# DataZooDE/anofox-forecast

Hardware: AMD Instinct MI355X
Metric: series/sec fit+forecast, AutoETS h=28 on M5-shape batches (higher is better)
Workload: dtype f64

## Files before the change

### anofox-forecast_amd/csrc/ets_group_kernel.hpp

```cpp
#pragma once
#include "fit_units.hpp"

namespace anofox {

template <int ID, int MSG> constexpr int group_member_ms()
{
    if constexpr (SpecOf<ID>::s == 0) return 0;
    else if constexpr (MSG == 12 && !SpecOf<ID>::Cfg::ADDITIVE) return -1;
    else return MSG;
}
template <int ID, int MSG> constexpr bool group_member_k4() { return SpecOf<ID>::Cfg::ADDITIVE && (group_member_ms<ID, MSG>() == 0 || group_member_ms<ID, MSG>() == 7); }

template <class YT, int... IDS> struct GroupTraits {
    static constexpr bool OK = ((RoundTraits<typename SpecOf<IDS>::Cfg, YT>::WAVES == RoundTraits<typename SpecOf<0>::Cfg, YT>::WAVES &&
                                 RoundTraits<typename SpecOf<IDS>::Cfg>::WPB == 1 && !RoundTraits<typename SpecOf<IDS>::Cfg>::PARK) && ...);
};

template <class YT> constexpr int group_waves = RoundTraits<typename SpecOf<0>::Cfg, YT>::WAVES;

template <int ID, int MSG, class YT>
__device__ __forceinline__ void ets_group_slot(const FitArgs &a, const int k4, const int vblock, const int vgrid, double *const lds)
{
    using Cfg = typename SpecOf<ID>::Cfg;
    constexpr int MS = group_member_ms<ID, MSG>();
    if constexpr (SpecOf<ID>::s != 0 && MSG == 0) return;
    else {
        if constexpr (group_member_k4<ID, MSG>())
            if (k4) { ets_round_body<Cfg, MS, 3, true, YT>(a, vblock, vgrid, 0, lds); return; }
        ets_round_body<Cfg, MS, 3, false, YT>(a, vblock, vgrid, 0, lds);
    }
}

template <int MSG, class YT, int... IDS>
__global__ __launch_bounds__(NM_BLOCK, group_waves<YT>) void ets_group_round_kernel(const FitArgs *__restrict__ tab, const GroupRoundArgs g)
{
    extern __shared__ double lds_all[];
    const int b = (int)blockIdx.x;
    int k = 0;
    while (k + 1 < g.n_slots && b >= g.start[k + 1]) k++;
    const FitArgs &a = *(const FitArgs *)((const __attribute__((address_space(4))) FitArgs *)tab + k);
    const int vblock = b - g.start[k], vgrid = g.start[k + 1] - g.start[k], id = g.spec[k], k4 = g.k4[k];
    (void)((id == IDS && (ets_group_slot<IDS, MSG, YT>(a, k4, vblock, vgrid, lds_all), true)) || ...);
}

template <int MSG, class YT, int... IDS>
void ets_group_round_launch(const FitArgs *tab, const GroupRoundArgs &g, int m, hipStream_t stream)
{
    const int blocks = g.start[g.n_slots];
    if (blocks <= 0) return;
    size_t lds_doubles = 0;
    ((lds_doubles = std::max(lds_doubles, (size_t)nm_lds_doubles<SpecOf<IDS>::Cfg::DIM>() +
                                              (group_member_ms<IDS, MSG>() == -1 ? (size_t)m * NM_BLOCK : 0))), ...);
    const size_t lds_bytes = sizeof(double) * lds_doubles;
    if (lds_bytes > 48 * 1024)
        anofox_check_attr(hipFuncSetAttribute((const void *)ets_group_round_kernel<MSG, YT, IDS...>, hipFuncAttributeMaxDynamicSharedMemorySize, (int)lds_bytes));
    hipLaunchKernelGGL((ets_group_round_kernel<MSG, YT, IDS...>), dim3(blocks), dim3(NM_BLOCK), lds_bytes, stream, tab, g);
}

template <int MSG, int... IDS> GroupLaunchFn group_launcher_of_yt(int yt)
{
    if constexpr (!GroupTraits<double, IDS...>::OK || !GroupTraits<float, IDS...>::OK) return nullptr;
    else {
        if (yt == YT_U16) {
            if constexpr (ets_u16_variant(MSG) && GroupTraits<unsigned short, IDS...>::OK) return &ets_group_round_launch<MSG, unsigned short, IDS...>;
            else return nullptr;
        }
        if (yt == YT_F32) return &ets_group_round_launch<MSG, float, IDS...>;
        return &ets_group_round_launch<MSG, double, IDS...>;
    }
}
template <int... IDS> GroupLaunchFn group_launcher_of(int m, int yt)
{
    if (m <= 1) return group_launcher_of_yt<0, IDS...>(yt);
    if (m == 7) return group_launcher_of_yt<7, IDS...>(yt);
    constexpr bool ring12 = ((SpecOf<IDS>::s != 0 && SpecOf<IDS>::Cfg::ADDITIVE) || ...);
    if (m == 12 && ring12) return group_launcher_of_yt<12, IDS...>(yt);
    if (m > ETS_LDS_PERIOD) return group_launcher_of_yt<-2, IDS...>(yt);
    return group_launcher_of_yt<-1, IDS...>(yt);
}

}
```

### anofox-forecast_amd/csrc/fit_group_additive.hip

```cpp
#include "ets_group_kernel.hpp"
namespace anofox {
GroupLaunchFn fit_group_additive(int m, int yt) { return group_launcher_of<0, 1, 3, 4, 6, 7>(m, yt); }
}
```

### anofox-forecast_amd/csrc/fit_group_damped_mul.hip

```cpp
#include "ets_group_kernel.hpp"
namespace anofox {
GroupLaunchFn fit_group_damped_mul(int m, int yt) { return group_launcher_of<12, 13, 14, 27, 29>(m, yt); }
}
```

### anofox-forecast_amd/csrc/fit_group_general.hip

```cpp
#include "ets_group_kernel.hpp"
namespace anofox {
GroupLaunchFn fit_group_general(int m, int yt) { return group_launcher_of<2, 5, 8, 9, 10, 11, 15, 17, 18, 20, 21, 23, 24, 26>(m, yt); }
}
```

### anofox-forecast_amd/csrc/host_api.hip

```cpp
#include <hip/hip_runtime.h>

#include <algorithm>
#include <cctype>
#include <atomic>
#include <memory>
#include <unordered_map>
#include <chrono>
#include <cmath>
#include <condition_variable>
#include <mutex>
#include <cstdio>
#include <cstdlib>
#include <cstring>
#include <limits>
#include <map>
#include <stdexcept>
#include <string>
#include <system_error>
#include <thread>
#include <vector>

#include "classic_device.hpp"
#include "host_semantics.hpp"
#include "kernels.hpp"
// ... 765 lines not shown
        }
        b->yc_cells = cells;
    }
    if (!b->d_misfit) b->d_misfit = dalloc<unsigned int>(2);
    HIPCHECK(hipMemsetAsync(b->d_misfit, 0, 2 * sizeof(unsigned int), st));
    launch_compact_block(b->d_y, b->ld, d_len, (int)b->n, (int)std::max<size_t>(b->t_max, 1), b->d_yc32, b->d_yc16, b->d_misfit, st);
    b->h_misfit[0] = b->h_misfit[1] = 1u;
    HIPCHECK(hipMemcpyAsync(b->h_misfit, b->d_misfit, sizeof b->h_misfit, hipMemcpyDeviceToHost, st));
    return true;
}
void compact_storage_decide(AnofoxHipBatch *b, bool pending, hipStream_t st, int m)
{
    b->y_type = YT_F64;
    if (!pending) return;
    HIPCHECK(hipStreamSynchronize(st));
    const bool u16_kernels = b->d_m_col == nullptr && (m <= 1 || m == 7);
    if (b->h_misfit[1] == 0u && b->tun.compact != 1 && u16_kernels) b->y_type = YT_U16;
    else if (b->h_misfit[0] == 0u) b->y_type = YT_F32;
}

static_assert(N_GROUP_CLASSES == FIT_GROUP_CLASSES && GROUP_DAMPED_MUL == 0 && GROUP_GENERAL == 1 && GROUP_ADDITIVE == 2, "host_fit_schedule.hpp names the group classes by number");
void launch_fit_slots(AnofoxHipBatch *b, const std::vector<int> &specs, const int32_t *d_len, int m, bool skip_constant,
                      hipStream_t st)
{
    const size_t n = b->n, ld = b->ld, n_spec = specs.size();
    HIPCHECK(hipEventRecord(b->ev_fit0, st));
    const bool merged = b->d_m_col != nullptr;
    const int yt = b->y_type;
    const void *ybase = yt == YT_F32 ? (const void *)b->d_yc32 : (yt == YT_U16 ? (const void *)b->d_yc16 : (const void *)b->d_y);
    const int ybytes = yt == YT_F32 ? 4 : (yt == YT_U16 ? 2 : 8);
    const int lds_limit = merged ? ETS_MERGED_LDS_PERIOD : ETS_LDS_PERIOD;
    std::vector<FitLaunchers> fns_of(n_spec);
    GroupLaunchFn group_fn[N_GROUP_CLASSES];
    FitScheduleInput in;
    in.n = n; in.ld = ld; in.t_max = b->t_max; in.m = m;
    for (size_t k = 0; k < n_spec; k++) {
        const int id = specs[k], ms = spec_season(id) != 0 ? m : 1;
        fns_of[k] = ets_fit_launcher(id, (merged && ms != 1) ? (ms > lds_limit ? ETS_PERLANE_HBM : ETS_PERLANE_LDS) : ms, yt);
        if (!fns_of[k].round_seq || !fns_of[k].round_spec || !fns_of[k].round_auto || !fns_of[k].final) throw HipFail{"no kernel for ETS spec id " + std::to_string(id)};
        in.specs.push_back(FitSpec{id, spec_has_mult(id), spec_trend_idx(id) == 4, spec_season(id) != 0, fns_of[k].round_k4 && fns_of[k].round_auto_k4,
                                   fns_of[k].nm_scratch_per_wg, ets_group_class(id)});
    }
    for (int c = 0; c < N_GROUP_CLASSES; c++) { group_fn[c] = ets_group_launcher(c, m, yt); in.group_launcher[c] = group_fn[c] != nullptr; }
    in.live_pos = b->live_pos; in.live_all = b->live_all; in.use_pos = b->use_pos; in.none_pos = b->none_pos;
    in.fixed_params = b->fixed_params; in.merged = merged; in.fp64 = yt == YT_F64; in.use_gather = b->use_gather; in.gather_budget = b->gather_budget;
    in.seq_rounds = b->seq_rounds; in.seq_rounds_env = b->seq_rounds_env;
    in.spec_below = b->spec_below; in.spec_below_md = b->spec_below_md; in.spec2_below = b->spec2_below; in.spec2_below_md = b->spec2_below_md;
    in.n_lanes = std::min<int>(N_AUX_STREAMS, b->n_slots_cap);
    {
        const Tunables &t = b->tun;
        in.budgets = t.budgets; in.k4 = t.k4; in.k4_top = t.k4_top; in.k4_top_below = t.k4_top_below;
        in.fill_policy = t.fill_policy; in.fill_target = t.fill_target; in.fill_late_div = t.fill_late_div; in.fill_s2_div = t.fill_s2_div;
        in.top_boost_n = t.top_boost_n; in.top_boost_pct = t.top_boost_pct; in.prio_top = t.prio_top;
        in.group_launch = t.group_launch; in.group_split = t.group_split; in.dm_head_rounds = t.dm_head_rounds; in.gather_cols = t.gather_cols;
    }
    in.lim = FitLimits{NM_BLOCK, NM_K, GROUP_MAX_SLOTS, N_AUX_STREAMS, TINY_BATCH_PROBLEMS, lds_limit, 2 * 1024 * 64};
    const FitSchedule plan = plan_fit_schedule(in);
    if (!plan.error.empty()) throw HipFail{plan.error};
    auto spec_stream = [&](size_t oi) -> hipStream_t { return plan.inline_stream ? st : b->aux[plan.stream_of[oi]]; };
    std::vector<FitArgs> args(n_spec);
    std::vector<FitLaunchers> fns(n_spec);
    for (size_t oi = 0; oi < n_spec; oi++) {
        const size_t k = plan.order[oi];
        const int id = specs[k];
        auto &lane = b->lanes[plan.lane_of[oi]];
        const int se = spec_season(id), ti = spec_trend_idx(id);
        const int tt = ti == 0 ? 0 : (ti <= 2 ? 1 : 2);
        FitArgs &a = args[oi];
        a = FitArgs{};
        a.y = (const double *)ybase; a.ld = ld; a.len = d_len; a.n_series = (int)n; a.t_rows = (int)std::max<size_t>(b->t_max, 1);
        a.m = se != 0 ? m : 1; a.h = b->h;
        a.l0 = b->d_l0 + (size_t)(se * 3 + tt) * ld;
        a.b0 = b->d_b0 + (size_t)(se * 3 + tt) * ld;
        a.fig = se == 1 ? b->d_fig_add : (se == 2 ? b->d_fig_mul : nullptr);
        a.fig_ld = ld;
        a.flags = b->d_flags;
        a.need_positive = spec_has_mult(id) ? 1 : 0;
        a.skip_constant = skip_constant ? 1 : 0;
        a.n_param = spec_n_param(id, a.m);
        a.aicc = b->d_aicc + k * ld;
        a.yhat = b->d_yhat_slots + k * n * (size_t)b->h;
        a.status = b->d_status_slots + k * ld;
        a.evals = b->d_evals_slots + k * ld;
        a.iters = b->d_iters_slots + k * ld;
        a.passes = b->d_passes_slots + k * ld;
        a.st = lane.st;
        a.ring_scratch = nullptr;
// ... 137 lines not shown
        hipStream_t sg = b->aux[plan.groups[g].stream];
        if (r == 0) {
            int32_t *zero[GROUP_MAX_SLOTS] = {};
            for (size_t k = 0; k < slots.size(); k++) zero[k] = b->lanes[plan.lane_of[slots[k]]].cnt;
            launch_group_zero3((int)slots.size(), zero, sg);
        }
        GroupCompactArgs gc{}; gc.n_series = (int)n;
        GroupGatherArgs gg{}; gg.t_max = (int)b->t_max; gg.elem_bytes = ybytes; gg.y = ybase; gg.ld = ld;
        int gg_cols = 0;
        GroupRoundArgs ga{};
        ga.n_slots = (int)slots.size();
        for (int k = 0; k < ga.n_slots; k++) {
            const size_t oi = slots[(size_t)k];
            const RoundStep &s = plan.steps[oi][(size_t)r];
            auto &lane = b->lanes[plan.lane_of[oi]];
            if (s.source == SRC_POSITIVE) retire_nonpositive(oi, sg);
            else if (s.source == SRC_COMPACTED) {
                const int c = gc.n_slots++;
                gc.prev[c] = (r == 1) ? nullptr : lane.map[(r - 1) & 1]; gc.n_prev[c] = (r == 1) ? nullptr : lane.cnt + ((r - 1) % 3); gc.done[c] = lane.st.done;
                gc.next[c] = lane.map[r & 1]; gc.n_next[c] = lane.cnt + (r % 3); gc.n_clear[c] = lane.cnt + ((r + 1) % 3);
                if (b->use_gather && lane.ybuf) {
                    const int j = gg.n_slots++;
                    gg.series_of[j] = lane.map[r & 1]; gg.n_active[j] = lane.cnt + (r % 3);
                    gg.out[j] = lane.ybuf; gg.ld_out[j] = lane.ybuf_cols; gg.cap[j] = (int)lane.ybuf_cols;
                    gg_cols = std::max(gg_cols, (int)std::min<size_t>(n, lane.ybuf_cols));
                }
            }
            ga.spec[k] = specs[plan.order[oi]];
            ga.k4[k] = s.k4 ? 1 : 0;
            ga.start[k + 1] = ga.start[k] + s.workgroups;
        }
        if (gc.n_slots > 0) launch_group_compact(gc, sg);
        if (gg.n_slots > 0) launch_group_gather(gg, gg_cols, sg);
        group_fn[plan.groups[g].cls](b->d_group_tab + (size_t)r * plan.n_slots + plan.slot_of[slots[0]], ga, m, sg);
        b->fit_launches++;
    };
    if (plan.head_rounds > 0) {
        for (int r = 0; r < plan.head_rounds; r++) {
            if (plan.grouped) enqueue_group_round(r, 0);
            else for (size_t oi = 0; oi < n_spec; oi++) if (plan.head[oi]) enqueue_round(r, oi);
        }
        LAUNCHCHECK("ETS fit head rounds");
        if (plan.grouped) {
            HIPCHECK(hipEventRecord(b->ev_join[0], b->aux[0]));
            for (size_t g = 1; g < plan.groups.size(); g++) HIPCHECK(hipStreamWaitEvent(b->aux[plan.groups[g].stream], b->ev_join[0], 0));
        } else {
            for (size_t od = 0; od < n_spec; od++) if (plan.head[od]) HIPCHECK(hipEventRecord(b->ev_join[plan.stream_of[od]], spec_stream(od)));
            for (size_t oi = 0; oi < n_spec; oi++) {
                if (plan.dead[oi] || plan.head[oi]) continue;
                for (size_t od = 0; od < n_spec; od++) if (plan.head[od]) HIPCHECK(hipStreamWaitEvent(spec_stream(oi), b->ev_join[plan.stream_of[od]], 0));
            }
        }
    }
    for (int r = 0; r < plan.total_rounds; r++) {
        const bool ahead = r < plan.head_rounds;
        if (plan.grouped) {
            for (size_t g = 0; g < plan.groups.size(); g++) if (!(ahead && plan.head[plan.groups[g].slots[0]])) enqueue_group_round(r, g);
        } else
            for (size_t oi = 0; oi < n_spec; oi++) if (!(ahead && plan.head[oi])) enqueue_round(r, oi);
        LAUNCHCHECK("ETS fit round");
    }
    if (b->fixed_params && n_spec == 1) HIPCHECK(hipEventRecord(b->ev_fit0, spec_stream(0)));
    for (size_t oi = 0; oi < n_spec; oi++) if (!plan.dead[oi]) fns[oi].final(args[oi], spec_stream(oi));
    if (b->fixed_params && n_spec == 1) HIPCHECK(hipEventRecord(b->ev_fit1, spec_stream(0)));
    LAUNCHCHECK("ETS final pass");
    for (int q : plan.fork_streams) {
        HIPCHECK(hipEventRecord(b->ev_join[q], b->aux[q]));
// ... 6979 lines not shown
```

### anofox-forecast_amd/csrc/host_fit_schedule.hpp

```cpp
#pragma once

enum RoundKind { RK_SEQ, RK_SPEC, RK_SPEC2, RK_AUTO, RK_K4, RK_AUTO_K4 };
enum SeriesSource { SRC_ALL, SRC_POSITIVE, SRC_COMPACTED };
constexpr int FIT_GROUP_CLASSES = 3;

struct FitLimits {
    int nm_block, nm_k;
    int group_max_slots;
    int n_aux_streams;
    int tiny_batch_problems;
    int lds_period;
    int64_t resident_lanes;
};

struct FitSpec {
    int id;
    bool has_mult, damped_mul, seasonal;
    bool has_k4;
    size_t nm_scratch_per_wg;
    int group_class;
};

struct FitScheduleInput {
    size_t n = 0, ld = 0, t_max = 0;
    int m = 1;
    std::vector<FitSpec> specs;
    int32_t live_pos = -1, live_all = -1;
    bool use_pos = false, none_pos = false, fixed_params = false, merged = false, fp64 = true, use_gather = false;
    double gather_budget = 0.0;
    int seq_rounds = 3, seq_rounds_env = -1;
    int spec_below = 8192, spec_below_md = 8192, spec2_below = 1024, spec2_below_md = 2048;
    int n_lanes = 1;
    std::vector<int> budgets;
    int k4 = -1, k4_top = 1, k4_top_below = 20480;
    int fill_policy = 1, fill_target = 150, fill_late_div = 2, fill_s2_div = 16;
    int top_boost_n = 0, top_boost_pct = 200, prio_top = 0;
    int group_launch = 1, group_split = 1, dm_head_rounds = 0, gather_cols = 0;
    bool group_launcher[FIT_GROUP_CLASSES] = {false, false, false};
    FitLimits lim{};
};

struct RoundStep {
    int kind;
    int budget, budget_seq;
    int spec_below, spec2_below;
    int wave_prio;
    int source;
    int workgroups;
    bool k4;
};

struct FitGroup { std::vector<size_t> slots; int stream; int cls; };

struct FitSchedule {
    std::string error;
    std::vector<size_t> order;
    std::vector<int> stream_of, lane_of;
    bool inline_stream = false;
    std::vector<int> fork_streams;
    std::vector<char> dead, k4, fill_spec4, head;
    bool fill_mode = false, tiny = false, grouped = false;
    int total_rounds = 0, head_rounds = 0;
    std::vector<FitGroup> groups;
    std::vector<size_t> slot_of;
    size_t n_slots = 0;
    size_t scratch_workgroups = 0;
    std::vector<size_t> gather_cols;
    std::vector<std::vector<RoundStep>> steps;
};

inline int fit_cost(int id)
{
    static const int measured[30] = { 3, 8, 14,  7, 13, 27,  17, 29, 41,  14, 26, 22,  63, 92, 84,
                                      7, 0, 15,  18, 0, 29,  33, 0, 48,  16, 0, 28,  65, 0, 95};
    return (id >= 0 && id < 30 && measured[id] > 0) ? measured[id] : 1;
}
inline double work(const FitScheduleInput &in, const FitSpec &s)
{
    const double live = (in.live_all >= 0 && s.has_mult) ? (double)in.live_pos : (in.live_all >= 0 ? (double)in.live_all : 1.0);
    return (double)fit_cost(s.id) * (live + 1.0);
}
inline int64_t live_problems(const FitScheduleInput &in, const FitSpec &s)
{
    return (s.has_mult && in.live_pos >= 0) ? (int64_t)in.live_pos : (in.live_all >= 0 ? (int64_t)in.live_all : (int64_t)in.n);
}
inline bool tiny_batch(const FitScheduleInput &in) { return (uint64_t)in.n * in.specs.size() <= (uint64_t)in.lim.tiny_batch_problems; }
inline size_t widest_launch_workgroups(const FitScheduleInput &in)
{
    const size_t n = in.n;
    return std::max<size_t>((n + 15) / 16, std::min<size_t>(n, tiny_batch(in) ? n : (size_t)std::max(in.spec2_below, in.spec2_below_md)));
}
inline int step_workgroups(const FitScheduleInput &in, const RoundStep &s)
{
    const int64_t n = (int64_t)in.n, per_spec = in.lim.nm_block / in.lim.nm_k;
    const int64_t g_seq = (n + in.lim.nm_block - 1) / in.lim.nm_block;
    if (s.kind == RK_SEQ || s.kind == RK_K4) return (int)g_seq;
// ... 82 lines not shown
            if (c < 0 || c >= FIT_GROUP_CLASSES || !in.group_launcher[c] || spec(oi).nm_scratch_per_wg != 0) p.grouped = false;
            else of_class[c].push_back(oi);
        }
        auto add = [&](const std::vector<size_t> &sl, int c) {
            if (sl.empty()) return;
            if (sl.size() > (size_t)in.lim.group_max_slots) p.error = "launch_fit_slots: more specs in one group than GROUP_MAX_SLOTS";
            p.groups.push_back(FitGroup{sl, 0, c});
        };
        auto add_class = [&](int c, bool split) {
            if (!split) { add(of_class[c], c); return; }
            std::vector<size_t> half[2];
            double w[2] = {0.0, 0.0};
            for (size_t oi : of_class[c]) {
                const int j = w[1] < w[0] ? 1 : 0;
                half[j].push_back(oi); w[j] += work(in, spec(oi));
            }
            add(half[0], c); add(half[1], c);
        };
        if (p.grouped) {
            add_class(0, in.group_split == 1);
            add_class(1, in.group_split == 2);
            add_class(2, false);
            if (!p.error.empty()) return p;
            p.grouped = !p.groups.empty();
        }
        for (size_t g = 0; g < p.groups.size(); g++) {
            const bool dm = spec(p.groups[g].slots[0]).damped_mul;
            p.groups[g].stream = dm ? (int)g : in.lim.n_aux_streams - 1 - (int)g;
            for (size_t oi : p.groups[g].slots) { p.stream_of[oi] = p.groups[g].stream; p.slot_of[oi] = p.n_slots++; }
        }
        if (p.grouped) for (size_t oi = 0; oi < n_spec; oi++) if (p.dead[oi]) p.stream_of[oi] = p.groups[0].stream;
    }
    if (p.grouped) for (const FitGroup &g : p.groups) p.fork_streams.push_back(g.stream);
    else if (!p.inline_stream) for (int i = 0; i < in.n_lanes; i++) p.fork_streams.push_back(i);
    p.head.assign(n_spec, 0);
    if (in.dm_head_rounds > 0 && p.total_rounds > 0 && !p.tiny && !p.inline_stream) {
        size_t n_dm = 0, n_rest = 0;
        if (p.grouped) {
            if (p.groups.size() > 1 && p.groups[0].stream == 0 && spec(p.groups[0].slots[0]).damped_mul) {
                for (size_t oi : p.groups[0].slots) p.head[oi] = 1;
                n_dm = n_rest = 1;
            }
        } else
            for (size_t oi = 0; oi < n_spec; oi++) {
                if (p.dead[oi]) continue;
                if (spec(oi).damped_mul) { p.head[oi] = 1; n_dm++; } else n_rest++;
            }
        if (n_dm && n_rest) p.head_rounds = std::min(in.dm_head_rounds, p.total_rounds);
        else p.head.assign(n_spec, 0);
    }
    p.steps.resize(n_spec);
    for (size_t oi = 0; oi < n_spec; oi++) {
        if (p.dead[oi]) continue;
        const FitSpec &sp = spec(oi);
        const int64_t live = live_problems(in, sp);
        const int s2 = sp.damped_mul ? in.spec2_below_md : in.spec2_below;
        for (int r = 0; r < p.total_rounds; r++) {
            RoundStep s{};
            s.wave_prio = (int)oi < in.prio_top ? std::max(1, 3 - (int)oi) : 0;
            s.spec_below = -1; s.spec2_below = -1;
            s.source = (p.tiny || (r == 0 && !(in.use_pos && sp.has_mult))) ? SRC_ALL : (r == 0 ? SRC_POSITIVE : SRC_COMPACTED);
            if (p.tiny) {
                s.kind = RK_SPEC2; s.budget = 1 << 30;
            } else if (p.fill_mode && !p.k4[oi]) {
                s.budget = BUDGET[r];
                if (r == 0) {
                    s.kind = p.fill_spec4[oi] ? RK_SPEC : RK_SEQ;
                    if (!p.fill_spec4[oi]) s.budget = (BUDGET[r] * 7) / 4;
                } else {
                    s.kind = RK_AUTO; s.budget_seq = (BUDGET[r] * 7) / 4;
                    s.spec_below = p.fill_spec4[oi] ? unconditional : (int)std::max<int64_t>(64, live / std::max(1, in.fill_late_div));
                    s.spec2_below = (int)std::max<int64_t>(32, std::min<int64_t>(s2 > 0 ? s2 : 32, live / std::max(1, in.fill_s2_div)));
                }
            } else if (p.k4[oi]) {
                const int sb = ((int)oi < in.k4_top && in.k4_top_below > 0) ? in.k4_top_below : in.spec_below;
                s.budget = BUDGET[r];
                if (r == 0) s.kind = live > sb ? RK_K4 : RK_SPEC;
                else { s.kind = RK_AUTO_K4; s.budget_seq = BUDGET[r]; s.spec_below = sb; s.spec2_below = s2 > 0 ? s2 : -1; }
            } else if (r == 0 || in.seq_rounds_env >= 0 || in.seq_rounds == 0) {
                const bool spec_mode = r >= in.seq_rounds;
                s.budget = spec_mode ? BUDGET[r] : (BUDGET[r] * 7) / 4;
                if (spec_mode && r > 0 && s2 > 0) { s.kind = RK_AUTO; s.budget_seq = s.budget; s.spec_below = unconditional; s.spec2_below = s2; }
                else s.kind = spec_mode ? RK_SPEC : RK_SEQ;
            } else {
                s.kind = RK_AUTO; s.budget = BUDGET[r]; s.budget_seq = (BUDGET[r] * 7) / 4;
                s.spec_below = sp.damped_mul ? in.spec_below_md : in.spec_below;
                s.spec2_below = s2 > 0 ? s2 : -1;
                if ((int)oi < in.top_boost_n) {
                    s.spec_below = (int)std::min<int64_t>(unconditional, (int64_t)s.spec_below * in.top_boost_pct / 100);
                    if (s.spec2_below > 0) s.spec2_below = (int)std::min<int64_t>(unconditional, (int64_t)s.spec2_below * in.top_boost_pct / 100);
                }
            }
            if (s.kind != RK_AUTO && s.kind != RK_AUTO_K4) s.budget_seq = s.budget;
            s.k4 = s.kind == RK_K4 || s.kind == RK_AUTO_K4;
            if (p.grouped) {
                if (s.kind == RK_SPEC) s.spec_below = unconditional;
                else if (s.kind == RK_SPEC2) { p.error = "launch_fit_slots: the one-wave-per-problem round of a tiny batch has no group form"; return p; }
            }
            s.workgroups = step_workgroups(in, s);
            if (p.grouped && sp.seasonal && in.m > in.lim.lds_period && (size_t)s.workgroups > p.scratch_workgroups) {
                p.error = "launch_fit_slots: the seasonal-ring scratch does not cover a group slot"; return p;
            }
            p.steps[oi].push_back(s);
        }
    }
    return p;
}
```

### anofox-forecast_amd/csrc/host_resources.hpp

```cpp
#pragma once

constexpr int N_AUX_STREAMS = 32;

struct HipFail { std::string msg; bool oom = false; };
void report_hip_failure(AnofoxError *out_error, const HipFail &f)
{
    if (f.oom) anofox::set_error(out_error, ALLOCATION_ERROR, "Allocation error: " + f.msg);
    else anofox::set_error(out_error, INTERNAL_ERROR, "Internal error: " + f.msg);
}
#define HIPCHECK(expr)                                                                             \
    do {                                                                                           \
        hipError_t _e = (expr);                                                                    \
        if (_e != hipSuccess) throw HipFail{std::string(#expr) + ": " + hipGetErrorString(_e), _e == hipErrorOutOfMemory};    \
    } while (0)

#define LAUNCHCHECK(what)                                                                          \
    do {                                                                                           \
        hipError_t _e = hipGetLastError();                                                         \
        if (_e != hipSuccess) throw HipFail{std::string("kernel launch failed (") + (what) + "): " + hipGetErrorString(_e), false};    \
    } while (0)

constexpr int32_t STATUS_NOT_COMPUTED = -1;

struct Tunables {
    std::vector<int> budgets{24, 24, 24, 24, 24, 24, 48, 48, 96, 96, 192, 1024};
    int seq_rounds = -1;
    int gather_cols = 0;
    int gather = -1;
    int spec_below = 8192;
    int spec_below_md = 8192;
    int spec2_below = 1024;
    int spec2_below_md = 2048;
    int k4 = -1;
    int k4_top = 1, k4_top_below = 20480;
    std::string wave_trace;
    int compact = -1;
    int fill_policy = 1;
    int fill_target = 150;
    int fill_late_div = 2;
    int fill_s2_div = 16;
    int top_boost_n = 0, top_boost_pct = 200;
    int prio_top = 0;
    int group_launch = 1;
    int group_split = 1;
    int dm_head_rounds = 0;
    bool merge_periods = true;
    int part_threads = 16;
    int pack_threads = 0;
    bool timing = false;
    int arima_trace = 0;
    double arima_lookahead = 6.0;
    int arima_lookahead_depth = 2;
    double arima_spec_factor = 4.0;
    double arima_shared_chunk_rounds = 1.0;
    int arima_prep_lanes = 64;
    int arima_queue_sort = 1;
    int arima_refit_budget = 100;
    static std::map<std::string, std::string> tune_map()
    {
        std::map<std::string, std::string> kv;
        const char *e = std::getenv("ANOFOX_HIP_TUNE");
        if (!e) return kv;
        std::string all(e);
        for (size_t pos = 0; pos < all.size();) {
            size_t end = all.find(';', pos);
            if (end == std::string::npos) end = all.size();
            const std::string item = all.substr(pos, end - pos);
            const size_t eq = item.find('=');
            if (eq != std::string::npos) {
                std::string k = item.substr(0, eq), v = item.substr(eq + 1);
                while (!k.empty() && k.front() == ' ') k.erase(k.begin());
                while (!k.empty() && k.back() == ' ') k.pop_back();
                kv[k] = v;
            }
            pos = end + 1;
        }
        return kv;
    }
    static Tunables from_env()
    {
        Tunables t;
        const std::map<std::string, std::string> kv = tune_map();
        auto geti = [&](const char *k, int &v) { auto it = kv.find(k); if (it != kv.end()) v = std::atoi(it->second.c_str()); };
        auto getd = [&](const char *k, double &v) { auto it = kv.find(k); if (it != kv.end()) v = std::atof(it->second.c_str()); };
        if (kv.count("budgets")) {
            std::vector<int> v;
            for (const char *q = kv.at("budgets").c_str(); *q;) {
                char *end = nullptr;
                long x = std::strtol(q, &end, 10);
                if (end == q) break;
                if (x > 0) v.push_back((int)x);
                q = (*end == ',') ? end + 1 : end;
            }
            if (!v.empty()) t.budgets = v;
        }
        if (kv.count("wave_trace")) t.wave_trace = kv.at("wave_trace");
        geti("compact", t.compact); geti("prio_top", t.prio_top); geti("top_boost_n", t.top_boost_n); geti("top_boost_pct", t.top_boost_pct);
        geti("fill_policy", t.fill_policy); geti("fill_target", t.fill_target); geti("fill_late_div", t.fill_late_div); geti("fill_s2_div", t.fill_s2_div);
        geti("seq_rounds", t.seq_rounds);
        geti("gather", t.gather);
        if (kv.count("spec_below")) t.spec_below = t.spec_below_md = std::atoi(kv.at("spec_below").c_str());
        geti("spec_below_md", t.spec_below_md);
        geti("gather_cols", t.gather_cols);
        geti("group_launch", t.group_launch); geti("group_split", t.group_split);
        geti("k4", t.k4); geti("dm_head_rounds", t.dm_head_rounds); geti("k4_top", t.k4_top); geti("k4_top_below", t.k4_top_below);
        if (kv.count("spec2_below")) t.spec2_below = t.spec2_below_md = std::atoi(kv.at("spec2_below").c_str());
        geti("spec2_below_md", t.spec2_below_md);
        if (kv.count("merge_periods")) t.merge_periods = std::atoi(kv.at("merge_periods").c_str()) != 0;
        geti("part_threads", t.part_threads);
        if (kv.count("arima_trace")) t.arima_trace = std::atoi(kv.at("arima_trace").c_str());
        getd("arima_lookahead", t.arima_lookahead);
        geti("arima_lookahead_depth", t.arima_lookahead_depth);
        getd("arima_spec_factor", t.arima_spec_factor);
        geti("arima_queue_sort", t.arima_queue_sort);
        geti("arima_prep_lanes", t.arima_prep_lanes);
        getd("arima_shared_chunk_rounds", t.arima_shared_chunk_rounds);
        geti("arima_refit_budget", t.arima_refit_budget);
        if (const char *e = std::getenv("ANOFOX_HIP_PACK_THREADS")) t.pack_threads = std::max(1, std::atoi(e));
        t.timing = std::getenv("ANOFOX_HIP_TIMING") != nullptr;
        return t;
    }
};
struct ProcessTunables {
    double cache_gb = -1.0, pinned_cache_gb = 2.0;
    double coalesce_us = 1000.0;
    int prio_streams = -1;
    std::string devices;
    static const ProcessTunables &get()
    {
        static const ProcessTunables t = [] {
            ProcessTunables p;
            if (const char *e = std::getenv("ANOFOX_HIP_CACHE_GB")) p.cache_gb = std::atof(e);
            if (const char *e = std::getenv("ANOFOX_HIP_PINNED_CACHE_GB")) p.pinned_cache_gb = std::atof(e);
            { const auto kv = Tunables::tune_map(); auto it = kv.find("prio_streams"); if (it != kv.end()) p.prio_streams = std::atoi(it->second.c_str()); }
            if (const char *e = std::getenv("ANOFOX_HIP_COALESCE_US")) p.coalesce_us = std::atof(e);
            if (const char *e = std::getenv("ANOFOX_HIP_DEVICES")) p.devices = e;
            return p;
        }();
// ... 425 lines not shown
```

### anofox-forecast_amd/csrc/kernels.hip

```cpp
#include "classic_device.hpp"
#include "fit_units.hpp"
#include "kernels.hpp"
#include "det_trig.hpp"
#include "../../include/anofox_fcst_hip.h"

namespace anofox {

__global__ __launch_bounds__(NM_BLOCK) void select_kernel(const SelectArgs a)
{
    const int s = blockIdx.x * NM_BLOCK + threadIdx.x;
    if (s >= a.n_series) return;
    if (a.len[s] <= 0) { a.fallback_mask[s] = 0u; return; }
    int best = -1;
    double best_aicc = __builtin_huge_val();
    int passes = 0, evals = 0;
    for (int k = 0; k < a.n_slots; k++) {
        passes += a.passes_slots[(size_t)k * a.ld + s];
        evals += a.evals_slots[(size_t)k * a.ld + s];
        if (a.status_slots[(size_t)k * a.ld + s] != FIT_OK) continue;
        double v = a.aicc[(size_t)k * a.ld + s];
        if (v < best_aicc) { best_aicc = v; best = k; }
    }
    a.passes_total[s] = passes;
    a.evals_total[s] = evals;
// ... 169 lines not shown
    hipLaunchKernelGGL(simple_kernel, dim3(grid), dim3(NM_BLOCK), 0, stream, a);
}

__global__ __launch_bounds__(256) void interval_kernel(const IntervalArgs a)
{
    const size_t idx = (size_t)blockIdx.x * 256 + threadIdx.x;
    const size_t total = (size_t)a.n_series * a.h;
    if (idx >= total) return;
    const int s = (int)(idx / a.h), i = (int)(idx % a.h);
    if (a.status[s] != 0) { a.lower[idx] = __builtin_nan(""); a.upper[idx] = __builtin_nan(""); return; }
    const double wd = a.z * a.sd[s] * sqrt((double)(i + 1));
    const double f = a.yhat[idx];
    a.lower[idx] = f - wd;
    a.upper[idx] = f + wd;
}

void launch_intervals(const IntervalArgs &a, hipStream_t stream)
{
    const size_t total = (size_t)a.n_series * a.h;
    if (total == 0) return;
    hipLaunchKernelGGL(interval_kernel, dim3((unsigned)((total + 255) / 256)), dim3(256), 0, stream, a);
}

FitLaunchers ets_fit_launcher(int spec_id, int m, int yt)
{
    FitLaunchers f = fit_unit_nonseasonal(spec_id, m, yt);
    if (!f.final) f = fit_unit_seasonal_add(spec_id, m, yt);
    if (!f.final) f = fit_unit_seasonal_gen_a(spec_id, m, yt);
    if (!f.final) f = fit_unit_seasonal_gen_m(spec_id, m, yt);
    return f;
}

GroupLaunchFn fit_group_damped_mul(int m, int yt);
GroupLaunchFn fit_group_general(int m, int yt);
GroupLaunchFn fit_group_additive(int m, int yt);
GroupLaunchFn ets_group_launcher(int group_class, int m, int yt)
{
    if (group_class == GROUP_DAMPED_MUL) return fit_group_damped_mul(m, yt);
    if (group_class == GROUP_GENERAL) return fit_group_general(m, yt);
    if (group_class == GROUP_ADDITIVE) return fit_group_additive(m, yt);
    return nullptr;
}

__global__ __launch_bounds__(NM_BLOCK) void compact_kernel(const int32_t *series_prev, const int32_t *n_prev_ptr, int n_series,
                                                           const int32_t *done, int32_t *series_next, int32_t *n_next_ptr, int32_t *n_clear)
{
    if (n_clear && blockIdx.x == 0 && threadIdx.x == 0) *n_clear = 0;
    const int n_prev = n_prev_ptr ? *n_prev_ptr : n_series;
    if ((int)blockIdx.x * NM_BLOCK >= n_prev) return;
    const int lane = threadIdx.x;
    const int idx = blockIdx.x * NM_BLOCK + lane;
    int s = 0;
    bool keep = false;
    if (idx < n_prev) {
        s = series_prev ? series_prev[idx] : idx;
        keep = done[s] == 0;
    }
    const unsigned long long bal = __ballot(keep);
    const int cnt = __popcll(bal);
    if (cnt == 0) return;
    int base = 0;
    if (lane == 0) base = atomicAdd(n_next_ptr, cnt);
    base = __shfl(base, 0);
    const int before = __popcll(bal & ((1ull << lane) - 1ull));
    if (keep) series_next[base + before] = s;
}

void launch_compact(const int32_t *series_prev, const int32_t *n_prev, int n_series, const int32_t *done,
                    int32_t *series_next, int32_t *n_next, hipStream_t stream, int32_t *n_clear)
{
    if (!n_clear) anofox_check_attr(hipMemsetAsync(n_next, 0, sizeof(int32_t), stream));
    const int grid = (n_series + NM_BLOCK - 1) / NM_BLOCK;
    hipLaunchKernelGGL(compact_kernel, dim3(grid), dim3(NM_BLOCK), 0, stream, series_prev, n_prev, n_series, done, series_next, n_next, n_clear);
}

// ... 303 lines not shown
```

### anofox-forecast_amd/csrc/kernels.hpp

```cpp
#pragma once
#include <hip/hip_runtime.h>
#include <stddef.h>
#include <stdint.h>
#include <atomic>

#include <stdexcept>
#include <string>

namespace anofox {

inline void anofox_check_attr(hipError_t e)
{
    if (e != hipSuccess) throw std::runtime_error(std::string("launch preparation failed: ") + hipGetErrorString(e));
}

enum : uint32_t { SF_POSITIVE = 1u, SF_CONSTANT = 2u, SF_HAS_NAN = 4u };

enum : int32_t { FIT_OK = 0, FIT_SHORT = 1, FIT_NONPOSITIVE = 2, FIT_NONFINITE = 3, FIT_PERIOD = 4, FIT_SKIPPED = 5 };

struct PrepArgs {
    const double *y; size_t ld; const int32_t *len; int n_series;
    int m;
    const int32_t *m_col;
    double *mean, *sd;
// ... 579 lines not shown
    size_t t_rows;
    const double *x;
    const double *f;
    double *yhat;
    int32_t *status;
    int32_t *model_code;
    double *b0, *beta;
    uint32_t *used;
};
void launch_exog_arimax(const ExogArgs &, hipStream_t);

struct IntervalArgs {
    int n_series, h;
    const double *yhat, *sd;
    const int32_t *status;
    double z;
    double *lower, *upper;
};

typedef void (*FitLaunchFn)(const FitArgs &, hipStream_t);
struct FitLaunchers { FitLaunchFn round_seq, round_spec, round_spec2, round_auto, final; size_t nm_scratch_per_wg; FitLaunchFn round_k4, round_auto_k4; };
constexpr int ETS_PERLANE_LDS = -3, ETS_PERLANE_HBM = -4;
FitLaunchers ets_fit_launcher(int spec_id, int m, int yt = 0);
constexpr int GROUP_MAX_SLOTS = 16;
enum { GROUP_DAMPED_MUL = 0, GROUP_GENERAL = 1, GROUP_ADDITIVE = 2, N_GROUP_CLASSES = 3 };
struct GroupRoundArgs {
    int n_slots;
    int spec[GROUP_MAX_SLOTS];
    int k4[GROUP_MAX_SLOTS];
    int start[GROUP_MAX_SLOTS + 1];
};
typedef void (*GroupLaunchFn)(const FitArgs *tab, const GroupRoundArgs &g, int m, hipStream_t);
GroupLaunchFn ets_group_launcher(int group_class, int m, int yt);
inline int ets_group_class(int spec_id)
{
    if (spec_id < 0 || spec_id >= 30 || (spec_id >= 15 && spec_id % 3 == 1)) return -1;
    const int e = spec_id / 15, ti = (spec_id % 15) / 3, s = spec_id % 3;
    if (ti == 4) return GROUP_DAMPED_MUL;
    return (e == 0 && ti < 3 && s < 2) ? GROUP_ADDITIVE : GROUP_GENERAL;
}
FitLaunchers classic_fit_launcher(int kind, int m);
struct ClassicArgs;
void launch_classic_final(int kind, const FitArgs &a, const ClassicArgs &c, hipStream_t stream);

struct GroupCompactArgs {
    int n_slots, n_series;
    const int32_t *prev[GROUP_MAX_SLOTS], *n_prev[GROUP_MAX_SLOTS], *done[GROUP_MAX_SLOTS];
    int32_t *next[GROUP_MAX_SLOTS], *n_next[GROUP_MAX_SLOTS], *n_clear[GROUP_MAX_SLOTS];
};
void launch_group_compact(const GroupCompactArgs &g, hipStream_t);
void launch_group_zero3(int n, int32_t *const *zero, hipStream_t);
struct GroupGatherArgs {
    int n_slots, t_max, elem_bytes;
    const void *y; size_t ld;
    const int32_t *series_of[GROUP_MAX_SLOTS], *n_active[GROUP_MAX_SLOTS];
    void *out[GROUP_MAX_SLOTS]; size_t ld_out[GROUP_MAX_SLOTS]; int cap[GROUP_MAX_SLOTS];
};
void launch_group_gather(const GroupGatherArgs &g, int n_cols_max, hipStream_t);
void launch_compact(const int32_t *series_prev, const int32_t *n_prev, int n_series, const int32_t *done,
                    int32_t *series_next, int32_t *n_next, hipStream_t, int32_t *n_clear = nullptr);
constexpr int DETECT_LDS_ROWS = 8192;
constexpr int DETECT_LONG_GRID = 1024;
size_t detect_scratch_doubles(int n_series, int t_rows);
void launch_detect_periods(const double *y, size_t ld, const int32_t *len, int n_series, int t_rows, double *scratch, int32_t *period,
                           double *best_acf, hipStream_t stream);
void launch_gather_columns(const void *y, size_t ld, const int32_t *series_of, const int32_t *n_active, int n_series,
// ... 121 lines not shown
```

Measured before the change: 79540.

## Add register-capped partner group kernels and optional solo damped-multiplicative kernel

Splits the grouped ETS round kernel into three variants. A partner variant caps VGPRs at 124 and is now used for the additive and general groups. A solo variant requests 132 VGPRs and pads its live registers, so that one solo wave plus one partner wave fill a SIMD's register file. A new schedule option can run the first rounds of the damped-multiplicative group with the solo kernel, optionally at higher wave priority, so the long-running class co-resides with the others rather than contending. The register cap on partner kernels applies by default and risks spills; the solo path is off unless tuned.

```diff
diff --git a/anofox-forecast_amd/csrc/ets_group_kernel.hpp b/anofox-forecast_amd/csrc/ets_group_kernel.hpp
--- a/anofox-forecast_amd/csrc/ets_group_kernel.hpp
+++ b/anofox-forecast_amd/csrc/ets_group_kernel.hpp
@@ -31,8 +31,16 @@
     }
 }
 
+enum { GROUP_PLACE_ANY = 0, GROUP_PLACE_PARTNER = 1, GROUP_PLACE_SOLO = 2 };
+constexpr int GROUP_SOLO_REGS = 264, GROUP_PARTNER_REGS = 248;
+#define ANOFOX_GROUP_PARTNER_NUM_VGPR 124
+#define ANOFOX_GROUP_SOLO_NUM_VGPR 132
+static_assert(2 * ANOFOX_GROUP_PARTNER_NUM_VGPR == GROUP_PARTNER_REGS && 2 * ANOFOX_GROUP_SOLO_NUM_VGPR == GROUP_SOLO_REGS &&
+              GROUP_SOLO_REGS > 256 && GROUP_SOLO_REGS % 8 == 0 && GROUP_PARTNER_REGS % 8 == 0 && GROUP_SOLO_REGS + GROUP_PARTNER_REGS <= 512,
+              "the solo and the partner allocation share one SIMD's 512 registers, in granules of 8");
+
 template <int MSG, class YT, int... IDS>
-__global__ __launch_bounds__(NM_BLOCK, group_waves<YT>) void ets_group_round_kernel(const FitArgs *__restrict__ tab, const GroupRoundArgs g)
+__device__ __forceinline__ void ets_group_round(const FitArgs *__restrict__ tab, const GroupRoundArgs &g)
 {
     extern __shared__ double lds_all[];
     const int b = (int)blockIdx.x;
@@ -44,6 +52,33 @@
 }
 
 template <int MSG, class YT, int... IDS>
+__global__ __launch_bounds__(NM_BLOCK, group_waves<YT>) void ets_group_round_kernel(const FitArgs *__restrict__ tab, const GroupRoundArgs g)
+{
+    ets_group_round<MSG, YT, IDS...>(tab, g);
+}
+
+template <int MSG, class YT, int... IDS>
+__global__ __launch_bounds__(NM_BLOCK, group_waves<YT>) __attribute__((amdgpu_num_vgpr(ANOFOX_GROUP_PARTNER_NUM_VGPR)))
+void ets_group_round_partner_kernel(const FitArgs *__restrict__ tab, const GroupRoundArgs g)
+{
+    ets_group_round<MSG, YT, IDS...>(tab, g);
+}
+
+template <int MSG, class YT> constexpr int group_solo_pad() { return MSG != 0 ? 8 : (sizeof(YT) == 8 ? 48 : 16); }
+template <int MSG, class YT, int... IDS>
+__global__ __launch_bounds__(NM_BLOCK, 1) __attribute__((amdgpu_num_vgpr(ANOFOX_GROUP_SOLO_NUM_VGPR)))
+void ets_group_round_solo_kernel(const FitArgs *__restrict__ tab, const GroupRoundArgs g)
+{
+    constexpr int PAD = group_solo_pad<MSG, YT>();
+    unsigned pad[PAD];
+#pragma unroll
+    for (int i = 0; i < PAD; i++) asm volatile("v_mov_b32 %0, 0" : "=v"(pad[i]));
+    ets_group_round<MSG, YT, IDS...>(tab, g);
+#pragma unroll
+    for (int i = 0; i < PAD; i++) asm volatile("" ::"v"(pad[i]));
+}
+
+template <int PLACE, int MSG, class YT, int... IDS>
 void ets_group_round_launch(const FitArgs *tab, const GroupRoundArgs &g, int m, hipStream_t stream)
 {
     const int blocks = g.start[g.n_slots];
@@ -52,31 +87,35 @@
     ((lds_doubles = std::max(lds_doubles, (size_t)nm_lds_doubles<SpecOf<IDS>::Cfg::DIM>() +
                                               (group_member_ms<IDS, MSG>() == -1 ? (size_t)m * NM_BLOCK : 0))), ...);
     const size_t lds_bytes = sizeof(double) * lds_doubles;
+    void (*kernel)(const FitArgs *, GroupRoundArgs) = nullptr;
+    if constexpr (PLACE == GROUP_PLACE_SOLO) kernel = ets_group_round_solo_kernel<MSG, YT, IDS...>;
+    else if constexpr (PLACE == GROUP_PLACE_PARTNER) kernel = ets_group_round_partner_kernel<MSG, YT, IDS...>;
+    else kernel = ets_group_round_kernel<MSG, YT, IDS...>;
     if (lds_bytes > 48 * 1024)
-        anofox_check_attr(hipFuncSetAttribute((const void *)ets_group_round_kernel<MSG, YT, IDS...>, hipFuncAttributeMaxDynamicSharedMemorySize, (int)lds_bytes));
-    hipLaunchKernelGGL((ets_group_round_kernel<MSG, YT, IDS...>), dim3(blocks), dim3(NM_BLOCK), lds_bytes, stream, tab, g);
+        anofox_check_attr(hipFuncSetAttribute((const void *)kernel, hipFuncAttributeMaxDynamicSharedMemorySize, (int)lds_bytes));
+    hipLaunchKernelGGL(kernel, dim3(blocks), dim3(NM_BLOCK), lds_bytes, stream, tab, g);
 }
 
-template <int MSG, int... IDS> GroupLaunchFn group_launcher_of_yt(int yt)
+template <int PLACE, int MSG, int... IDS> GroupLaunchFn group_launcher_of_yt(int yt)
 {
     if constexpr (!GroupTraits<double, IDS...>::OK || !GroupTraits<float, IDS...>::OK) return nullptr;
     else {
         if (yt == YT_U16) {
-            if constexpr (ets_u16_variant(MSG) && GroupTraits<unsigned short, IDS...>::OK) return &ets_group_round_launch<MSG, unsigned short, IDS...>;
+            if constexpr (ets_u16_variant(MSG) && GroupTraits<unsigned short, IDS...>::OK) return &ets_group_round_launch<PLACE, MSG, unsigned short, IDS...>;
             else return nullptr;
         }
-        if (yt == YT_F32) return &ets_group_round_launch<MSG, float, IDS...>;
-        return &ets_group_round_launch<MSG, double, IDS...>;
+        if (yt == YT_F32) return &ets_group_round_launch<PLACE, MSG, float, IDS...>;
+        return &ets_group_round_launch<PLACE, MSG, double, IDS...>;
     }
 }
-template <int... IDS> GroupLaunchFn group_launcher_of(int m, int yt)
+template <int PLACE, int... IDS> GroupLaunchFn group_launcher_of(int m, int yt)
 {
-    if (m <= 1) return group_launcher_of_yt<0, IDS...>(yt);
-    if (m == 7) return group_launcher_of_yt<7, IDS...>(yt);
+    if (m <= 1) return group_launcher_of_yt<PLACE, 0, IDS...>(yt);
+    if (m == 7) return group_launcher_of_yt<PLACE, 7, IDS...>(yt);
     constexpr bool ring12 = ((SpecOf<IDS>::s != 0 && SpecOf<IDS>::Cfg::ADDITIVE) || ...);
-    if (m == 12 && ring12) return group_launcher_of_yt<12, IDS...>(yt);
-    if (m > ETS_LDS_PERIOD) return group_launcher_of_yt<-2, IDS...>(yt);
-    return group_launcher_of_yt<-1, IDS...>(yt);
+    if (m == 12 && ring12) return group_launcher_of_yt<PLACE, 12, IDS...>(yt);
+    if (m > ETS_LDS_PERIOD) return group_launcher_of_yt<PLACE, -2, IDS...>(yt);
+    return group_launcher_of_yt<PLACE, -1, IDS...>(yt);
 }
 
 }
diff --git a/anofox-forecast_amd/csrc/fit_group_additive.hip b/anofox-forecast_amd/csrc/fit_group_additive.hip
--- a/anofox-forecast_amd/csrc/fit_group_additive.hip
+++ b/anofox-forecast_amd/csrc/fit_group_additive.hip
@@ -1,4 +1,4 @@
 #include "ets_group_kernel.hpp"
 namespace anofox {
-GroupLaunchFn fit_group_additive(int m, int yt) { return group_launcher_of<0, 1, 3, 4, 6, 7>(m, yt); }
+GroupLaunchFn fit_group_additive(int m, int yt) { return group_launcher_of<GROUP_PLACE_PARTNER, 0, 1, 3, 4, 6, 7>(m, yt); }
 }
diff --git a/anofox-forecast_amd/csrc/fit_group_damped_mul.hip b/anofox-forecast_amd/csrc/fit_group_damped_mul.hip
--- a/anofox-forecast_amd/csrc/fit_group_damped_mul.hip
+++ b/anofox-forecast_amd/csrc/fit_group_damped_mul.hip
@@ -1,4 +1,4 @@
 #include "ets_group_kernel.hpp"
 namespace anofox {
-GroupLaunchFn fit_group_damped_mul(int m, int yt) { return group_launcher_of<12, 13, 14, 27, 29>(m, yt); }
+GroupLaunchFn fit_group_damped_mul(int m, int yt) { return group_launcher_of<GROUP_PLACE_ANY, 12, 13, 14, 27, 29>(m, yt); }
 }
diff --git a/anofox-forecast_amd/csrc/fit_group_damped_mul_solo.hip b/anofox-forecast_amd/csrc/fit_group_damped_mul_solo.hip
--- /dev/null
+++ b/anofox-forecast_amd/csrc/fit_group_damped_mul_solo.hip
@@ -0,0 +1,4 @@
+#include "ets_group_kernel.hpp"
+namespace anofox {
+GroupLaunchFn fit_group_damped_mul_solo(int m, int yt) { return group_launcher_of<GROUP_PLACE_SOLO, 12, 13, 14, 27, 29>(m, yt); }
+}
diff --git a/anofox-forecast_amd/csrc/fit_group_general.hip b/anofox-forecast_amd/csrc/fit_group_general.hip
--- a/anofox-forecast_amd/csrc/fit_group_general.hip
+++ b/anofox-forecast_amd/csrc/fit_group_general.hip
@@ -1,4 +1,4 @@
 #include "ets_group_kernel.hpp"
 namespace anofox {
-GroupLaunchFn fit_group_general(int m, int yt) { return group_launcher_of<2, 5, 8, 9, 10, 11, 15, 17, 18, 20, 21, 23, 24, 26>(m, yt); }
+GroupLaunchFn fit_group_general(int m, int yt) { return group_launcher_of<GROUP_PLACE_PARTNER, 2, 5, 8, 9, 10, 11, 15, 17, 18, 20, 21, 23, 24, 26>(m, yt); }
 }
diff --git a/anofox-forecast_amd/csrc/host_api.hip b/anofox-forecast_amd/csrc/host_api.hip
--- a/anofox-forecast_amd/csrc/host_api.hip
+++ b/anofox-forecast_amd/csrc/host_api.hip
@@ -821,6 +821,7 @@
     const int lds_limit = merged ? ETS_MERGED_LDS_PERIOD : ETS_LDS_PERIOD;
     std::vector<FitLaunchers> fns_of(n_spec);
     GroupLaunchFn group_fn[N_GROUP_CLASSES];
+    const GroupLaunchFn solo_fn = ets_group_solo_launcher(m, yt);
     FitScheduleInput in;
     in.n = n; in.ld = ld; in.t_max = b->t_max; in.m = m;
     for (size_t k = 0; k < n_spec; k++) {
@@ -842,6 +843,7 @@
         in.fill_policy = t.fill_policy; in.fill_target = t.fill_target; in.fill_late_div = t.fill_late_div; in.fill_s2_div = t.fill_s2_div;
         in.top_boost_n = t.top_boost_n; in.top_boost_pct = t.top_boost_pct; in.prio_top = t.prio_top;
         in.group_launch = t.group_launch; in.group_split = t.group_split; in.dm_head_rounds = t.dm_head_rounds; in.gather_cols = t.gather_cols;
+        in.dm_solo_rounds = t.dm_solo_rounds; in.dm_solo_prio = t.dm_solo_prio; in.dm_solo_launcher = solo_fn != nullptr;
     }
     in.lim = FitLimits{NM_BLOCK, NM_K, GROUP_MAX_SLOTS, N_AUX_STREAMS, TINY_BATCH_PROBLEMS, lds_limit, 2 * 1024 * 64};
     const FitSchedule plan = plan_fit_schedule(in);
@@ -1045,7 +1047,7 @@
         }
         if (gc.n_slots > 0) launch_group_compact(gc, sg);
         if (gg.n_slots > 0) launch_group_gather(gg, gg_cols, sg);
-        group_fn[plan.groups[g].cls](b->d_group_tab + (size_t)r * plan.n_slots + plan.slot_of[slots[0]], ga, m, sg);
+        (plan.solo[g][(size_t)r] ? solo_fn : group_fn[plan.groups[g].cls])(b->d_group_tab + (size_t)r * plan.n_slots + plan.slot_of[slots[0]], ga, m, sg);
         b->fit_launches++;
     };
     if (plan.head_rounds > 0) {
diff --git a/anofox-forecast_amd/csrc/host_fit_schedule.hpp b/anofox-forecast_amd/csrc/host_fit_schedule.hpp
--- a/anofox-forecast_amd/csrc/host_fit_schedule.hpp
+++ b/anofox-forecast_amd/csrc/host_fit_schedule.hpp
@@ -37,6 +37,8 @@
     int top_boost_n = 0, top_boost_pct = 200, prio_top = 0;
     int group_launch = 1, group_split = 1, dm_head_rounds = 0, gather_cols = 0;
     bool group_launcher[FIT_GROUP_CLASSES] = {false, false, false};
+    int dm_solo_rounds = 0, dm_solo_prio = 0;
+    bool dm_solo_launcher = false;
     FitLimits lim{};
 };
 
@@ -62,6 +64,7 @@
     bool fill_mode = false, tiny = false, grouped = false;
     int total_rounds = 0, head_rounds = 0;
     std::vector<FitGroup> groups;
+    std::vector<std::vector<char>> solo;
     std::vector<size_t> slot_of;
     size_t n_slots = 0;
     size_t scratch_workgroups = 0;
@@ -210,6 +213,14 @@
         if (p.grouped) for (size_t oi = 0; oi < n_spec; oi++) if (p.dead[oi]) p.stream_of[oi] = p.groups[0].stream;
     }
     if (p.grouped) for (const FitGroup &g : p.groups) p.fork_streams.push_back(g.stream);
+    if (p.grouped) {
+        bool other_class = false;
+        for (const FitGroup &g : p.groups) if (g.cls != 0) other_class = true;
+        p.solo.assign(p.groups.size(), std::vector<char>((size_t)p.total_rounds, 0));
+        for (size_t g = 0; g < p.groups.size(); g++)
+            for (int r = 0; r < p.total_rounds; r++)
+                p.solo[g][(size_t)r] = p.groups[g].cls == 0 && r < in.dm_solo_rounds && in.dm_solo_launcher && other_class;
+    }
     else if (!p.inline_stream) for (int i = 0; i < in.n_lanes; i++) p.fork_streams.push_back(i);
     p.head.assign(n_spec, 0);
     if (in.dm_head_rounds > 0 && p.total_rounds > 0 && !p.tiny && !p.inline_stream) {
@@ -275,6 +286,7 @@
                 if (s.kind == RK_SPEC) s.spec_below = unconditional;
                 else if (s.kind == RK_SPEC2) { p.error = "launch_fit_slots: the one-wave-per-problem round of a tiny batch has no group form"; return p; }
             }
+            if (p.grouped && in.dm_solo_prio > 0 && sp.group_class == 0 && !p.solo.empty() && p.solo[0][(size_t)r]) s.wave_prio = in.dm_solo_prio;
             s.workgroups = step_workgroups(in, s);
             if (p.grouped && sp.seasonal && in.m > in.lim.lds_period && (size_t)s.workgroups > p.scratch_workgroups) {
                 p.error = "launch_fit_slots: the seasonal-ring scratch does not cover a group slot"; return p;
diff --git a/anofox-forecast_amd/csrc/host_resources.hpp b/anofox-forecast_amd/csrc/host_resources.hpp
--- a/anofox-forecast_amd/csrc/host_resources.hpp
+++ b/anofox-forecast_amd/csrc/host_resources.hpp
@@ -44,6 +44,8 @@
     int group_launch = 1;
     int group_split = 1;
     int dm_head_rounds = 0;
+    int dm_solo_rounds = 0;
+    int dm_solo_prio = 0;
     bool merge_periods = true;
     int part_threads = 16;
     int pack_threads = 0;
@@ -103,7 +105,7 @@
         geti("spec_below_md", t.spec_below_md);
         geti("gather_cols", t.gather_cols);
         geti("group_launch", t.group_launch); geti("group_split", t.group_split);
-        geti("k4", t.k4); geti("dm_head_rounds", t.dm_head_rounds); geti("k4_top", t.k4_top); geti("k4_top_below", t.k4_top_below);
+        geti("k4", t.k4); geti("dm_head_rounds", t.dm_head_rounds); geti("dm_solo_rounds", t.dm_solo_rounds); geti("dm_solo_prio", t.dm_solo_prio); geti("k4_top", t.k4_top); geti("k4_top_below", t.k4_top_below);
         if (kv.count("spec2_below")) t.spec2_below = t.spec2_below_md = std::atoi(kv.at("spec2_below").c_str());
         geti("spec2_below_md", t.spec2_below_md);
         if (kv.count("merge_periods")) t.merge_periods = std::atoi(kv.at("merge_periods").c_str()) != 0;
diff --git a/anofox-forecast_amd/csrc/kernels.hip b/anofox-forecast_amd/csrc/kernels.hip
--- a/anofox-forecast_amd/csrc/kernels.hip
+++ b/anofox-forecast_amd/csrc/kernels.hip
@@ -225,6 +225,7 @@
 }
 
 GroupLaunchFn fit_group_damped_mul(int m, int yt);
+GroupLaunchFn fit_group_damped_mul_solo(int m, int yt);
 GroupLaunchFn fit_group_general(int m, int yt);
 GroupLaunchFn fit_group_additive(int m, int yt);
 GroupLaunchFn ets_group_launcher(int group_class, int m, int yt)
@@ -234,6 +235,7 @@
     if (group_class == GROUP_ADDITIVE) return fit_group_additive(m, yt);
     return nullptr;
 }
+GroupLaunchFn ets_group_solo_launcher(int m, int yt) { return fit_group_damped_mul_solo(m, yt); }
 
 __global__ __launch_bounds__(NM_BLOCK) void compact_kernel(const int32_t *series_prev, const int32_t *n_prev_ptr, int n_series,
                                                            const int32_t *done, int32_t *series_next, int32_t *n_next_ptr, int32_t *n_clear)
diff --git a/anofox-forecast_amd/csrc/kernels.hpp b/anofox-forecast_amd/csrc/kernels.hpp
--- a/anofox-forecast_amd/csrc/kernels.hpp
+++ b/anofox-forecast_amd/csrc/kernels.hpp
@@ -635,6 +635,7 @@
 };
 typedef void (*GroupLaunchFn)(const FitArgs *tab, const GroupRoundArgs &g, int m, hipStream_t);
 GroupLaunchFn ets_group_launcher(int group_class, int m, int yt);
+GroupLaunchFn ets_group_solo_launcher(int m, int yt);
 inline int ets_group_class(int spec_id)
 {
     if (spec_id < 0 || spec_id >= 30 || (spec_id >= 15 && spec_id % 3 == 1)) return -1;
```

New measurement: 78620. 0.988x the previous value.
